# dylkot/cNMF

Measured on AMD Instinct MI355X. Metric: NMF restarts/sec (50000x2000xK5..13), higher is better.
Workload: dtype f32 (exact integer f16 plane x 2 f16 planes with per-row exponent, f32 accumulate)

## Files before the change

cnmf_amd/csrc/kernels_gemm2h.hip.h:

```cpp
#pragma once
#include <hip/hip_runtime.h>
#include "kernels_gemm3.hip.h"
#include "kernels_planes.hip.h"

namespace cnmf {

typedef _Float16 f16x8 __attribute__((ext_vector_type(8)));
typedef float f32x4_g __attribute__((ext_vector_type(4)));
typedef _Float16 f16x2_g __attribute__((ext_vector_type(2)));

#ifndef G2_U8_SKIP
#define G2_U8_SKIP 0
#endif

constexpr int G2_ROWB = 64;
constexpr int G2_A = G3_MW * G2_ROWB;
constexpr int G2_B = G3C_JW * 32;

template <int NSUB, bool HI, bool U8 = false>
struct G2Geom {
    static_assert(NSUB == 1 || (NSUB == 2 && !HI), "two blocks per step: one count plane only");
    static_assert(!U8 || NSUB == 2, "the byte plane is read by the 16x16x32 body only");
    static constexpr int IMGS = NSUB == 1 ? 4 : 3;
    static constexpr int IMG = U8 ? NSUB * G2_A + G2_B : NSUB * (G2_A + (HI ? 2 : 1) * G2_B);
    static constexpr int OFF_B = NSUB * G2_A, OFF_H = OFF_B + NSUB * G2_B;
    static constexpr int NA = NSUB * 2, NB = U8 ? 1 : NSUB;
    static constexpr int AHEAD = IMGS - 1;
    static constexpr int LDS_BYTES = IMGS * IMG;
};

template <int NSUB, bool U8 = false> struct G2Sub {};

#define G2_DMA_PIECE(NSUB_, HI_, NTB_, s_, i_)                                                     \
    {                                                                                              \
        using GEO_ = G2Geom<NSUB_, HI_>;                                                           \
        unsigned char* d_ = smem + ((s_) % GEO_::IMGS) * GEO_::IMG + wave * 1024;                  \
        if ((i_) < GEO_::NA)                                                                       \
            __builtin_amdgcn_global_load_lds(G3_AS1(abase + (size_t)(s_) * ((NSUB_) * G2_A) + (i_) * 8192), \
                                             G3_AS3(d_ + (i_) * 8192), 16, 0, 0);                  \
        else if ((i_) < GEO_::NA + GEO_::NB)    \
            __builtin_amdgcn_global_load_lds(G3_AS1(bbase + (size_t)(s_) * ((NSUB_) * G2_B) + ((i_) - GEO_::NA) * 8192), \
                                             G3_AS3(d_ + GEO_::OFF_B + ((i_) - GEO_::NA) * 8192), 16, 0, (NTB_) ? 2 : 0); \
        else if constexpr (HI_)                                                                    \
            __builtin_amdgcn_global_load_lds(G3_AS1(hbase + (size_t)(s_) * ((NSUB_) * G2_B) + ((i_) - GEO_::NA - GEO_::NB) * 8192), \
                                             G3_AS3(d_ + GEO_::OFF_H + ((i_) - GEO_::NA - GEO_::NB) * 8192), 16, 0, (NTB_) ? 2 : 0); \
    }

template <bool PART>
__device__ __forceinline__ unsigned g2_wave_live(unsigned live, int grp)
{
    return PART ? (unsigned)__builtin_amdgcn_readfirstlane((int)((live >> (grp * 4)) & 0xfu)) : 0xfu;
}


template <int VAR, bool NTB, bool PART, bool U8 = false>
__device__ __forceinline__ void gemm2h_segment_mf16(const unsigned char* __restrict__ A2, const unsigned char* __restrict__ B1,
                                                    const float* __restrict__ rscale, int Kb, float* __restrict__ C,
                                                    int ldc, int m0, int j0, int kb0, int nkb, unsigned char* smem,
                                                    unsigned live)
{
    static_assert(VAR == 0 || VAR == 2 || VAR == 3 || VAR == 4 || VAR == 6 || VAR == 7, "instruction streams 1 and 5 were retired");
    static_assert(!U8 || VAR == 0 || VAR == 4, "the byte plane has the burst and the spread stream only");
    using GEO = G2Geom<2, false, U8>;
    constexpr int NSUB = 2, IMGS = GEO::IMGS, IMG = GEO::IMG, OFF_B = GEO::OFF_B, NA = GEO::NA, NB = GEO::NB, AHEAD = GEO::AHEAD;
    constexpr bool BURST = VAR == 0, NOMFMA = VAR == 2, NODMA = VAR == 3 || VAR == 6 || VAR == 7;
    constexpr bool NOREAD = VAR == 6 || VAR == 7, NOBAR = VAR == 7;
    static_assert(IMGS == 3 && NA + NB == (U8 ? 5 : 6), "three images, six pieces per step (bytes: five)");
    const int tid = threadIdx.x;
    const int lane = tid & 63, wave = tid >> 6;
    const int grp = wave >> 2, wn = wave & 3;
    const int r = lane & 15, g = lane >> 4;
    const int ub = g >> 1, hf = g & 1;
    const int nst = nkb / NSUB;
    const unsigned lv = g2_wave_live<PART>(live, grp);
#define G2_LIVE(mt_) (!PART || ((lv >> ((mt_) >> 1)) & 1u))

    const unsigned char* abase = A2 + ((size_t)(m0 / G3_MW) * Kb + kb0) * G2_A + tid * 16;
    const unsigned char* bbase = U8 ? B1 + ((size_t)(j0 / G3C_JW) * (Kb / NSUB) + kb0 / NSUB) * G2_B + tid * 16
                                    : B1 + ((size_t)(j0 / G3C_JW) * Kb + kb0) * G2_B + tid * 16;
    constexpr const unsigned char* hbase = nullptr;

    f32x4_g acc[8][4];
#pragma unroll
    for (int mt = 0; mt < 8; ++mt)
#pragma unroll
        for (int nt = 0; nt < 4; ++nt)
#pragma unroll
            for (int i = 0; i < 4; ++i) acc[mt][nt][i] = 0.f;

    const int a_row = ub * G2_A + (grp * 128 + r) * G2_ROWB;
    const int a_s0 = ((0 + hf) ^ ((r >> 2) & 3)) * 16, a_s1 = ((2 + hf) ^ ((r >> 2) & 3)) * 16;
    const int b_off = U8 ? OFF_B + wn * 2048 + lane * 16 : OFF_B + ub * G2_B + (wn * 64 + r) * 32 + (hf ^ ((r >> 3) & 1)) * 16;

#define G2_DMA_PIECE_U8(s_, i_)                                                                    \
    {                                                                                              \
        unsigned char* d_ = smem + ((s_) % IMGS) * IMG + wave * 1024;                              \
        if ((i_) < NA)                                                                             \
            __builtin_amdgcn_global_load_lds(G3_AS1(abase + (size_t)(s_) * (NSUB * G2_A) + (i_) * 8192), \
                                             G3_AS3(d_ + (i_) * 8192), 16, 0, 0);                  \
        else                                                                                       \
            __builtin_amdgcn_global_load_lds(G3_AS1(bbase + (size_t)(s_) * G2_B), G3_AS3(d_ + OFF_B), 16, 0, NTB ? 2 : 0); \
    }
#define G2_PIECE(s_, i_) { if constexpr (U8) G2_DMA_PIECE_U8(s_, i_) else G2_DMA_PIECE(2, false, NTB, s_, i_) __builtin_amdgcn_sched_barrier(0); }
#define G2_SPOT(MORE_, p_)                                                                         \
    if (!BURST && MORE_) {                                                                         \
        if constexpr (!U8) G2_PIECE(s + AHEAD, p_)                                                 \
        else if constexpr ((p_) != G2_U8_SKIP) G2_PIECE(s + AHEAD, (p_) < G2_U8_SKIP ? (p_) : (p_) - 1) \
    }
#define G2_CVT2(w_, sel_) __builtin_bit_cast(unsigned, __builtin_bit_cast(f16x2_g, __builtin_amdgcn_perm(0x64646464u, (w_), (sel_))) - f16x2_g{(_Float16)1024.0f, (_Float16)1024.0f})
#define G2_SEL_LO 0x04010400u
#define G2_SEL_HI 0x04030402u
#define G2_CVT(nt_)                                                                                \
    {                                                                                              \
        const unsigned w0_ = braw[(nt_) >> 1][2 * ((nt_) & 1)], w1_ = braw[(nt_) >> 1][2 * ((nt_) & 1) + 1]; \
        u32x4 c_;                                                                                  \
        c_.x = G2_CVT2(w0_, G2_SEL_LO); c_.y = G2_CVT2(w0_, G2_SEL_HI);                            \
        c_.z = G2_CVT2(w1_, G2_SEL_LO); c_.w = G2_CVT2(w1_, G2_SEL_HI);                            \
        bq[nt_] = __builtin_bit_cast(f16x8, c_);                                                   \
    }
#define G2_ISSUE(s_) { _Pragma("unroll") for (int i = 0; i < NA + NB; ++i) G2_PIECE(s_, i) }
#define G2_FRAG(ptr_) __builtin_bit_cast(f16x8, *reinterpret_cast<const u32x4*>(ptr_))
#define G2_AFRAG(bb_, mt_, q_) G2_FRAG((bb_) + a_row + (mt_) * 16 * G2_ROWB + ((q_) ? a_s1 : a_s0))
#define G2_READ_A(s_)                                                                              \
    {                                                                                              \
        const unsigned char* bb = smem + ((s_) % IMGS) * IMG;                                      \
        if constexpr (U8) { _Pragma("unroll") for (int p = 0; p < 2; ++p) braw[p] = *reinterpret_cast<const u32x4*>(bb + b_off + p * 1024); } \
        else { _Pragma("unroll") for (int nt = 0; nt < 4; ++nt) bq[nt] = G2_FRAG(bb + b_off + nt * 16 * 32); } \
        _Pragma("unroll") for (int mp = 0; mp < 4; mp += 2) {                                      \
            aq[mp][1] = G2_AFRAG(bb, mp, 1); aq[mp + 1][1] = G2_AFRAG(bb, mp + 1, 1);              \
            aq[mp][0] = G2_AFRAG(bb, mp, 0); aq[mp + 1][0] = G2_AFRAG(bb, mp + 1, 0);              \
        }                                                                                          \
        __builtin_amdgcn_sched_barrier(0);                                                         \
         \
        if constexpr (U8) { _Pragma("unroll") for (int nt = 0; nt < 4; ++nt) G2_CVT(nt) }          \
    }
#define G2_READ_B(s_)                                                                              \
    {                                                                                              \
        const unsigned char* bb = smem + ((s_) % IMGS) * IMG;                                      \
        _Pragma("unroll") for (int mp = 4; mp < 8; mp += 2) {                                      \
            aq[mp][1] = G2_AFRAG(bb, mp, 1); aq[mp + 1][1] = G2_AFRAG(bb, mp + 1, 1);              \
            aq[mp][0] = G2_AFRAG(bb, mp, 0); aq[mp + 1][0] = G2_AFRAG(bb, mp + 1, 0);              \
        }                                                                                          \
        __builtin_amdgcn_sched_barrier(0);                                                         \
    }
#define G2_MF(mt_, q_)                                                                             \
    if constexpr (NOMFMA) { asm volatile("" :: "v"(aq[mt_][q_]), "v"(bq[0]), "v"(bq[1]), "v"(bq[2]), "v"(bq[3])); } \
    else if (G2_LIVE(mt_)) {                                                                       \
        _Pragma("unroll") for (int nt = 0; nt < 4; ++nt)                                           \
            acc[mt_][nt] = __builtin_amdgcn_mfma_f32_16x16x32_f16(aq[mt_][q_], bq[nt], acc[mt_][nt], 0, 0, 0); \
    }
#define G2_MF8(ma_, mb_, q_) G2_MF(ma_, q_) G2_MF(mb_, q_)
#define G2_STEP(MORE_)                                                                             \
    {                                                                                              \
        if constexpr (!NOBAR) G3_RAW_BARRIER()                   \
        if (BURST && MORE_) G2_ISSUE(s + AHEAD)                                                    \
        if constexpr (NOREAD) { if (s == 0) { G2_READ_A(s) G2_READ_B(s) } } else { G2_READ_A(s) }  \
        G2_MF8(0, 1, 1)                                                                            \
        G2_SPOT(MORE_, 0)                                                                          \
        G2_MF8(0, 1, 0)                                                                            \
        if constexpr (!NOREAD) { G2_READ_B(s) }                                                    \
        G2_SPOT(MORE_, 1)                                                                          \
        G2_MF8(2, 3, 1)                                                                            \
        G2_SPOT(MORE_, 2)                                                                          \
        G2_MF8(2, 3, 0)                                                                            \
        asm volatile("s_waitcnt lgkmcnt(0)" ::: "memory");       \
                                          \
        if (s + 1 < nst) {                                                                         \
            if (MORE_) {                                                                           \
                if constexpr (U8) { if constexpr (BURST) G3_WAIT_VM(5); else if constexpr (G2_U8_SKIP < 3) G3_WAIT_VM(2); else G3_WAIT_VM(3); } \
                else { if constexpr (BURST) G3_WAIT_VM(6); else G3_WAIT_VM(3); }                   \
            } else G3_WAIT_VM(0);                                                                  \
        }                                                                                          \
        if constexpr (!NOBAR) G3_RAW_BARRIER()                                            \
        G2_MF8(4, 5, 1)                                                                            \
        G2_SPOT(MORE_, 3)                                                                          \
        G2_MF8(4, 5, 0)                                                                            \
        G2_SPOT(MORE_, 4)                                                                          \
        G2_MF8(6, 7, 1)                                                                            \
        G2_SPOT(MORE_, 5)                                                                          \
        G2_MF8(6, 7, 0)                                                                            \
    }

    f16x8 bq[4], aq[8][2];
    u32x4 braw[2];
    G3_WAIT_VM(0);
    G2_ISSUE(0)
    if (nst > 1) G2_ISSUE(1)
    if (nst > 1) { if constexpr (U8) G3_WAIT_VM(5); else G3_WAIT_VM(6); } else G3_WAIT_VM(0);
    if (grp == 1) G3_RAW_BARRIER()
    {
        int s = 0;
        const int n_main = NODMA ? 0 : nst - AHEAD;
        for (; s < n_main; ++s) G2_STEP(true)
        for (; s < nst; ++s) G2_STEP(false)
    }
    if (grp == 0) G3_RAW_BARRIER()
#undef G2_STEP
#undef G2_MF8
#undef G2_MF
#undef G2_READ_B
#undef G2_READ_A
#undef G2_AFRAG
#undef G2_FRAG
#undef G2_ISSUE
#undef G2_CVT
#undef G2_SEL_HI
#undef G2_SEL_LO
#undef G2_CVT2
#undef G2_SPOT
#undef G2_PIECE
#undef G2_DMA_PIECE_U8

    if (C == nullptr) return;
#pragma unroll
    for (int mt = 0; mt < 8; ++mt) {
        if (!G2_LIVE(mt)) continue;
        const int row0 = m0 + grp * 128 + mt * 16 + 4 * g;
#pragma unroll
        for (int i = 0; i < 4; ++i) {
            const float rs = rscale[row0 + i];
#pragma unroll
            for (int nt = 0; nt < 4; ++nt)
                C[(size_t)(row0 + i) * ldc + j0 + wn * 64 + nt * 16 + r] = acc[mt][nt][i] * rs;
        }
    }
#undef G2_LIVE
}

template <bool HI, int VAR, bool NTB, bool PART, bool GEN>
__device__ __forceinline__ void gemm2h_segment(G2Sub<1>, const unsigned char* __restrict__ A2, const unsigned char* __restrict__ B1,
                                                   const unsigned char* __restrict__ Bhi,
                                                   const unsigned int* __restrict__ hiflag,
                                                   const float* __restrict__ rscale,
                                                   int Kb, float* __restrict__ C, int ldc, int m0, int j0, int kb0,
                                                   int nkb, unsigned char* smem, const float* __restrict__ cscale,
                                                   unsigned live)
{
    static_assert(VAR == 0 || VAR == 4, "the 32x32x16 body has the burst and the spread stream only");
    using GEO = G2Geom<1, HI>;
    constexpr int IMGS = GEO::IMGS, IMG = GEO::IMG, OFF_B = GEO::OFF_B, AHEAD = GEO::AHEAD;
    static_assert(IMGS == 4 && GEO::NA == 2 && GEO::NB == 1, "four images, pieces A0 A1 B (Bhi)");
    const int tid = threadIdx.x;
    const int lane = tid & 63, wave = tid >> 6;
    const int grp = wave >> 2, wn = wave & 3;
    const int li = lane & 31, h = lane >> 5;
    const int nst = nkb;
    const unsigned lv = g2_wave_live<PART>(live, grp);
#define G2_LIVE(m_) (!PART || ((lv >> (m_)) & 1u))

    const size_t jblk = ((size_t)(j0 / G3C_JW) * Kb + kb0);
    const unsigned char* abase = A2 + ((size_t)(m0 / G3_MW) * Kb + kb0) * G2_A + tid * 16;
    const unsigned char* bbase = B1 + jblk * G2_B + tid * 16;
    const unsigned char* hbase = HI ? Bhi + jblk * G2_B + tid * 16 : nullptr;
    unsigned int fw[5] = {0u, 0u, 0u, 0u, 0u};
    if (HI) {
        const int KW = (Kb + 31) >> 5, w0 = kb0 >> 5;
        const unsigned int* fr = hiflag + (size_t)(j0 / G3C_JW) * KW;
#pragma unroll
        for (int w = 0; w < 5; ++w)
            fw[w] = (nkb > 129) ? 0xFFFFFFFFu : ((w0 + w < KW) ? __builtin_amdgcn_readfirstlane(fr[w0 + w]) : 0u);
    }
    const int fbit0 = kb0 & 31;

    f32x16_3 acc[4][2];
#pragma unroll
    for (int m = 0; m < 4; ++m)
#pragma unroll
        for (int n = 0; n < 2; ++n)
#pragma unroll
            for (int r = 0; r < 16; ++r) acc[m][n][r] = 0.f;

    const int a_row = (grp * 128 + li) * G2_ROWB;
    const int a_s0 = ((0 + h) ^ ((li >> 2) & 3)) * 16, a_s1 = ((2 + h) ^ ((li >> 2) & 3)) * 16;
    const int b_off = OFF_B + (wn * 64 + li) * 32 + (h ^ ((li >> 3) & 1)) * 16;

#define G2_BLKFLAG(b_) (HI && ((fw[(fbit0 + (b_)) >> 5 > 4 ? 4 : (fbit0 + (b_)) >> 5] >> ((fbit0 + (b_)) & 31)) & 1u))
#define G2_ISSUE(s_)                                                                               \
    {                                                                                              \
        unsigned char* d_ = smem + ((s_) % IMGS) * IMG + wave * 1024;                              \
        const unsigned char* a_ = abase + (size_t)(s_) * G2_A;                                     \
        _Pragma("unroll") for (int i = 0; i < 2; ++i)                                              \
            __builtin_amdgcn_global_load_lds(G3_AS1(a_ + i * 8192), G3_AS3(d_ + i * 8192), 16, 0, 0); \
        __builtin_amdgcn_global_load_lds(G3_AS1(bbase + (size_t)(s_) * G2_B), G3_AS3(d_ + OFF_B), 16, 0, NTB ? 2 : 0); \
        if (HI) {                                                                                  \
            if (G2_BLKFLAG(s_))                                                                    \
                __builtin_amdgcn_global_load_lds(G3_AS1(hbase + (size_t)(s_) * G2_B), G3_AS3(d_ + GEO::OFF_H), 16, 0, NTB ? 2 : 0); \
        }                                                                                          \
    }
#define G2_PIECE(s_, i_) { G2_DMA_PIECE(1, HI, NTB, s_, i_) __builtin_amdgcn_sched_barrier(0); }
#define G2_FRAG(ptr_) __builtin_bit_cast(f16x8, *reinterpret_cast<const u32x4*>(ptr_))
#define G2_MFMA(b_, m_, q_)                                                                        \
    if (G2_LIVE(m_)) {                                                                             \
    acc[m_][0] = __builtin_amdgcn_mfma_f32_32x32x16_f16(aq[m_][q_], b_[0], acc[m_][0], 0, 0, 0);   \
    acc[m_][1] = __builtin_amdgcn_mfma_f32_32x32x16_f16(aq[m_][q_], b_[1], acc[m_][1], 0, 0, 0); }
#define G2_WAIT_AHEAD(cnt_)                                                                        \
    {                                                                                              \
        if constexpr ((cnt_) == 1) G3_WAIT_VM(3);                                                  \
        else if constexpr ((cnt_) == 2) G3_WAIT_VM(6);                                             \
        else G3_WAIT_VM(0);                                                                        \
    }

    f16x8 bq[2], bh[2], aq[4][2];
    constexpr bool SPREAD = VAR == 4 && (!HI || GEN);
    G3_WAIT_VM(0);
    G2_ISSUE(0)
    if (nst > 1) G2_ISSUE(1)
    if (nst > 2) G2_ISSUE(2)
    if (nst > 2) G2_WAIT_AHEAD(2) else if (nst > 1) G2_WAIT_AHEAD(1) else G2_WAIT_AHEAD(0)
    if (grp == 1) G3_RAW_BARRIER()
    if constexpr (SPREAD) {
#define G2_READ_A(s_)                                                                              \
        {                                                                                          \
            const unsigned char* bb = smem + ((s_) % IMGS) * IMG;                                  \
            _Pragma("unroll") for (int n = 0; n < 2; ++n) bq[n] = G2_FRAG(bb + b_off + n * 32 * 32); \
            _Pragma("unroll") for (int m = 0; m < 2; ++m) {                                        \
                aq[m][1] = G2_FRAG(bb + a_row + m * 32 * G2_ROWB + a_s1);                          \
                aq[m][0] = G2_FRAG(bb + a_row + m * 32 * G2_ROWB + a_s0);                          \
            }                                                                                      \
            if constexpr (HI) { _Pragma("unroll") for (int n = 0; n < 2; ++n) bh[n] = G2_FRAG(bb + b_off + G2_B + n * 32 * 32); } \
            __builtin_amdgcn_sched_barrier(0);                                                     \
        }
#define G2_READ_B(s_)                                                                              \
        {                                                                                          \
            const unsigned char* bb = smem + ((s_) % IMGS) * IMG;                                  \
            _Pragma("unroll") for (int m = 2; m < 4; ++m) {                                        \
                aq[m][1] = G2_FRAG(bb + a_row + m * 32 * G2_ROWB + a_s1);                          \
                aq[m][0] = G2_FRAG(bb + a_row + m * 32 * G2_ROWB + a_s0);                          \
            }                                                                                      \
            __builtin_amdgcn_sched_barrier(0);                                                     \
        }
#define G2_STEP(MORE_)                                                                             \
        {                                                                                          \
            G3_RAW_BARRIER()                                         \
            G2_READ_A(s)                                                                           \
            G2_MFMA(bq, 0, 1) G2_MFMA(bq, 1, 1)                                                    \
            if (MORE_) G2_PIECE(s + AHEAD, 0)                                                      \
            G2_MFMA(bq, 0, 0) G2_MFMA(bq, 1, 0)                                                    \
            G2_READ_B(s)                                                                           \
            if (MORE_) G2_PIECE(s + AHEAD, 1)                                                      \
            if constexpr (HI) { G2_MFMA(bh, 0, 0) G2_MFMA(bh, 1, 0) }                              \
            asm volatile("s_waitcnt lgkmcnt(0)" ::: "memory");                                     \
             \
            if (s + 1 < nst) { if (MORE_) { if constexpr (HI) G3_WAIT_VM(6); else G3_WAIT_VM(5); } else G3_WAIT_VM(0); } \
            G3_RAW_BARRIER()                                                              \
            G2_MFMA(bq, 2, 1) G2_MFMA(bq, 3, 1)                                                    \
            if (MORE_) G2_PIECE(s + AHEAD, 2)                                                      \
            G2_MFMA(bq, 2, 0) G2_MFMA(bq, 3, 0)                                                    \
            if constexpr (HI) { if (MORE_) G2_PIECE(s + AHEAD, 3)                                  \
                                G2_MFMA(bh, 2, 0) G2_MFMA(bh, 3, 0) }                              \
        }
        {
            int s = 0;
            const int n_main = nst - AHEAD;
            for (; s < n_main; ++s) G2_STEP(true)
            for (; s < nst; ++s) G2_STEP(false)
        }
#undef G2_STEP
#undef G2_READ_B
#undef G2_READ_A
    } else {
#define G2_READ(s_)                                                                                \
        {                                                                                          \
            const unsigned char* bb = smem + ((s_) % IMGS) * IMG;                                  \
            _Pragma("unroll") for (int n = 0; n < 2; ++n) bq[n] = G2_FRAG(bb + b_off + n * 32 * 32); \
            if (HI) { _Pragma("unroll") for (int n = 0; n < 2; ++n) bh[n] = G2_FRAG(bb + b_off + G2_B + n * 32 * 32); } \
            _Pragma("unroll") for (int m = 0; m < 4; ++m) {                                        \
                aq[m][0] = G2_FRAG(bb + a_row + m * 32 * G2_ROWB + a_s0);                          \
                aq[m][1] = G2_FRAG(bb + a_row + m * 32 * G2_ROWB + a_s1);                          \
            }                                                                                      \
            __builtin_amdgcn_sched_barrier(0);                                                     \
        }
#define G2_MFMA4(b_, ma_, mb_) G2_MFMA(b_, ma_, 1) G2_MFMA(b_, mb_, 1) G2_MFMA(b_, ma_, 0) G2_MFMA(b_, mb_, 0)
#define G2_MFMA2H(b_, ma_, mb_) G2_MFMA(b_, ma_, 0) G2_MFMA(b_, mb_, 0)
#define G2_HALF(ma_, mb_)                                                                          \
        {                                                                                          \
            G2_MFMA4(bq, ma_, mb_)                                                                 \
            if (HI) { if (hi_blk) { if constexpr (GEN) { G2_MFMA2H(bh, ma_, mb_) } else { G2_MFMA4(bh, ma_, mb_) } } } \
        }
        for (int s = 0; s < nst; ++s) {
            const bool hi_blk = G2_BLKFLAG(s);
            G3_RAW_BARRIER()
            if (s + AHEAD < nst) G2_ISSUE(s + AHEAD)
            G2_READ(s)
            G2_HALF(0, 1)
            asm volatile("s_waitcnt lgkmcnt(0)" ::: "memory");
            if (s + 1 < nst) {
                if (s + 3 < nst) G2_WAIT_AHEAD(2) else if (s + 2 < nst) G2_WAIT_AHEAD(1) else G2_WAIT_AHEAD(0)
            }
            G3_RAW_BARRIER()
            G2_HALF(2, 3)
        }
#undef G2_HALF
#undef G2_MFMA2H
#undef G2_MFMA4
#undef G2_READ
    }
    if (grp == 0) G3_RAW_BARRIER()
#undef G2_WAIT_AHEAD
#undef G2_MFMA
#undef G2_FRAG
#undef G2_PIECE
#undef G2_ISSUE
#undef G2_BLKFLAG

    if (C == nullptr) return;
    const int j = j0 + wn * 64 + li;
    const float cs[2] = {(HI && cscale) ? cscale[j] : 1.0f, (HI && cscale) ? cscale[j + 32] : 1.0f};
#pragma unroll
    for (int m = 0; m < 4; ++m) {
        if (!G2_LIVE(m)) continue;
        const int cbase = m0 + grp * 128 + m * 32 + 4 * h;
#pragma unroll
        for (int n = 0; n < 2; ++n)
#pragma unroll
            for (int r = 0; r < 16; ++r) {
                const int row = cbase + (r & 3) + 8 * (r >> 2);
                C[(size_t)row * ldc + j + n * 32] = (acc[m][n][r] * rscale[row]) * cs[n];
            }
    }
#undef G2_LIVE
}

template <bool HI, int VAR, bool NTB, bool PART, bool GEN, bool U8>
__device__ __forceinline__ void gemm2h_segment(G2Sub<2, U8>, const unsigned char* __restrict__ A2, const unsigned char* __restrict__ B1,
                                               const unsigned char* __restrict__, const unsigned int* __restrict__,
                                               const float* __restrict__ rscale, int Kb, float* __restrict__ C, int ldc,
                                               int m0, int j0, int kb0, int nkb, unsigned char* smem, const float* __restrict__,
                                               unsigned live)
{
    static_assert(!HI && !GEN, "two blocks per step: one count plane only");
    gemm2h_segment_mf16<VAR, NTB, PART, U8>(A2, B1, rscale, Kb, C, ldc, m0, j0, kb0, nkb, smem, live);
}

template <int NSUB, bool HI, int VAR = 0, bool PART = false, bool GEN = false, bool U8 = false>
__global__ __launch_bounds__(512) void gemm2h_kernel(const unsigned char* __restrict__ A2,
                                                     const unsigned char* __restrict__ B1,
                                                     const unsigned char* __restrict__ Bhi,
                                                     const unsigned int* __restrict__ hiflag,
                                                     const float* __restrict__ rscale, int Kb,
                                                     float* __restrict__ C, int ldc, long long c_split_stride,
                                                     int kb_per, const float* __restrict__ cscale = nullptr,
                                                     unsigned long long livemask = ~0ull)
{
    extern __shared__ __attribute__((aligned(16))) unsigned char smem3[];
    int jt = blockIdx.x, mg = blockIdx.y, z = blockIdx.z;
    if ((gridDim.z & 7) == 0) {
        const int L = blockIdx.x + (int)gridDim.x * (blockIdx.y + (int)gridDim.y * blockIdx.z);
        const int xcd = L & 7, idx = L >> 3;
        jt = idx % (int)gridDim.x;
        mg = (idx / (int)gridDim.x) % (int)gridDim.y;
        z = xcd + 8 * (idx / (int)(gridDim.x * gridDim.y));
    }
    const int kb0 = z * kb_per;
    const int nkb = min(kb_per, Kb - kb0);
    gemm2h_segment<HI, VAR, true, PART, GEN>(G2Sub<NSUB, U8>{}, A2, B1, Bhi, hiflag, rscale, Kb, C ? C + (size_t)z * c_split_stride : nullptr, ldc, mg * G3_MW,
                                                   jt * G3C_JW, kb0, nkb, smem3, cscale, (unsigned)((livemask >> (8 * mg)) & 0xffu));
}

template <int NSUB, bool HI, int VAR = 0, bool NTB = true, bool PART = false, bool GEN = false, bool U8 = false>
__global__ __launch_bounds__(512) void gemm2h_streamk_kernel(const unsigned char* __restrict__ A2,
                                                             const unsigned char* __restrict__ B1,
                                                             const unsigned char* __restrict__ Bhi,
                                                             const unsigned int* __restrict__ hiflag,
                                                             const float* __restrict__ rscale, int Kb,
                                                             float* __restrict__ C0, float* __restrict__ C1,
                                                             float* __restrict__ C2, int ldc, int MG, int T, int xmap,
                                                             const float* __restrict__ cscale = nullptr,
                                                             unsigned long long livemask = ~0ull)
{
    extern __shared__ __attribute__((aligned(16))) unsigned char smem3[];
    const int Ks = Kb / NSUB;
    const long long U = (long long)T * Ks;
    const int P = (int)gridDim.x;
    const int q = (xmap && MG > 1 && P % MG == 0) ? ((int)blockIdx.x % MG) * (P / MG) + (int)blockIdx.x / MG : (int)blockIdx.x;
    long long u = U * q / P;
    const long long u1 = U * (q + 1) / P;
    const int NJ = T / MG;
    while (u < u1) {
        const int tile = (int)(u / Ks), ks = (int)(u % Ks);
        const int ke = (int)min((long long)Ks, ks + (u1 - u));
        const int mg = tile / NJ, jt = tile % NJ;
        gemm2h_segment<HI, VAR, NTB, PART, GEN>(G2Sub<NSUB, U8>{}, A2, B1, Bhi, hiflag, rscale, Kb, (ks == 0) ? C0 : (ke == Ks ? C1 : C2), ldc, mg * G3_MW,
                                                      jt * G3C_JW, ks * NSUB, (ke - ks) * NSUB, smem3, cscale,
                                                      (unsigned)((livemask >> (8 * mg)) & 0xffu));
        u += ke - ks;
        G3_WAIT_VM(0);
        __syncthreads();
    }
}

}
```

Before: 236.5.

## Permute MFMA fragment rows to remove LDS bank conflicts in the 16x16 gemm body

Adds a constexpr helper header that models ds_read_b128 bank conflicts and defines permuted row mappings for the factor and count fragments. The 16x16x32 body now reads LDS rows through these permutations, and the epilogue remaps output rows and columns to match. The default U8 skip piece also changes from 0 to 2. The aim is fewer LDS bank conflicts on fragment reads. The cost is extra index arithmetic and a scattered output store pattern, and correctness depends on the permutation being consistent between reads and writes.

New measurement: 238.8 (median of 6 runs). Within noise of the previous version (+1.0%).

```diff
diff --git a/cnmf_amd/csrc/g2_frag.h b/cnmf_amd/csrc/g2_frag.h
--- /dev/null
+++ b/cnmf_amd/csrc/g2_frag.h
@@ -0,0 +1,76 @@
+#pragma once
+
+#include <cstdint>
+
+namespace g2frag {
+
+constexpr int ROWB = 64, A_BYTES = 256 * ROWB, B_BYTES = 256 * 32;
+constexpr int MF16_OFF_B = 2 * A_BYTES;
+constexpr int M32_OFF_B = A_BYTES;
+
+constexpr int b128_lane_group(int lane)
+{
+    const int l = lane & 31;
+    const bool first = l < 4 || (l >= 12 && l < 16) || (l >= 20 && l < 28);
+    return (lane >> 5) * 2 + (first ? 0 : 1);
+}
+
+template <class Off>
+constexpr int b128_extra_cycles(Off off)
+{
+    int extra = 0;
+    for (int grp = 0; grp < 4; ++grp) {
+        int worst = 0;
+        for (int bank = 0; bank < 16; ++bank) {
+            int addr[16] = {}, n = 0;
+            for (int lane = 0; lane < 64; ++lane) {
+                if (b128_lane_group(lane) != grp) continue;
+                const int a = off(lane);
+                if (((a >> 4) & 15) != bank) continue;
+                bool seen = false;
+                for (int i = 0; i < n; ++i) seen = seen || addr[i] == a;
+                if (!seen) addr[n++] = a;
+            }
+            worst = n > worst ? n : worst;
+        }
+        extra += worst - 1;
+    }
+    return extra;
+}
+
+constexpr int mf16_sigma(int t) { return (0x1320 >> (4 * t)) & 3; }
+constexpr int mf16_factor_row(int r) { return 4 * mf16_sigma(r >> 2) + (r & 3); }
+constexpr int mf16_count_row(int r) { return r ^ ((r & 8) >> 1); }
+
+constexpr int mf16_factor_off(int lane, int grp, int mt, int q, bool permuted = true)
+{
+    const int r = lane & 15, g = lane >> 4, ub = g >> 1, hf = g & 1;
+    const int row = permuted ? mf16_factor_row(r) : r;
+    return ub * A_BYTES + (grp * 128 + mt * 16 + row) * ROWB + (((2 * q + hf) ^ ((row >> 2) & 3)) * 16);
+}
+
+constexpr int mf16_count_off(int lane, int wn, int nt, bool permuted = true)
+{
+    const int r = lane & 15, g = lane >> 4, ub = g >> 1, hf = g & 1;
+    const int row = permuted ? mf16_count_row(r) : r;
+    return MF16_OFF_B + ub * B_BYTES + (wn * 64 + nt * 16 + row) * 32 + ((hf ^ ((row >> 3) & 1)) * 16);
+}
+
+constexpr int mf16_count_u8_off(int lane, int wn, int p) { return MF16_OFF_B + wn * 2048 + p * 1024 + lane * 16; }
+
+constexpr int mf16_out_row(int g, int mt, int i) { return mt * 16 + 4 * mf16_sigma(g) + i; }
+constexpr int mf16_out_col(int r, int nt, bool u8) { return nt * 16 + (u8 ? r : mf16_count_row(r)); }
+
+constexpr int m32_factor_off(int lane, int grp, int m, int q)
+{
+    const int li = lane & 31, h = lane >> 5;
+    return (grp * 128 + m * 32 + li) * ROWB + (((2 * q + h) ^ ((li >> 2) & 3)) * 16);
+}
+
+constexpr int m32_count_off(int lane, int wn, int n, int plane)
+{
+    const int li = lane & 31, h = lane >> 5;
+    return M32_OFF_B + plane * B_BYTES + (wn * 64 + n * 32 + li) * 32 + ((h ^ ((li >> 3) & 1)) * 16);
+}
+
+}
diff --git a/cnmf_amd/csrc/kernels_gemm2h.hip.h b/cnmf_amd/csrc/kernels_gemm2h.hip.h
--- a/cnmf_amd/csrc/kernels_gemm2h.hip.h
+++ b/cnmf_amd/csrc/kernels_gemm2h.hip.h
@@ -2,6 +2,7 @@
 #include <hip/hip_runtime.h>
 #include "kernels_gemm3.hip.h"
 #include "kernels_planes.hip.h"
+#include "g2_frag.h"
 
 namespace cnmf {
 
@@ -10,12 +11,17 @@
 typedef _Float16 f16x2_g __attribute__((ext_vector_type(2)));
 
 #ifndef G2_U8_SKIP
-#define G2_U8_SKIP 0
+#define G2_U8_SKIP 2
+#endif
+
+#ifndef G2_U8_PERMUTE
+#define G2_U8_PERMUTE 1
 #endif
 
 constexpr int G2_ROWB = 64;
 constexpr int G2_A = G3_MW * G2_ROWB;
 constexpr int G2_B = G3C_JW * 32;
+static_assert(g2frag::ROWB == G2_ROWB && g2frag::A_BYTES == G2_A && g2frag::B_BYTES == G2_B, "g2_frag.h restates this geometry");
 
 template <int NSUB, bool HI, bool U8 = false>
 struct G2Geom {
@@ -88,9 +94,12 @@
 #pragma unroll
             for (int i = 0; i < 4; ++i) acc[mt][nt][i] = 0.f;
 
-    const int a_row = ub * G2_A + (grp * 128 + r) * G2_ROWB;
-    const int a_s0 = ((0 + hf) ^ ((r >> 2) & 3)) * 16, a_s1 = ((2 + hf) ^ ((r >> 2) & 3)) * 16;
-    const int b_off = U8 ? OFF_B + wn * 2048 + lane * 16 : OFF_B + ub * G2_B + (wn * 64 + r) * 32 + (hf ^ ((r >> 3) & 1)) * 16;
+    constexpr bool PERM = !U8 || G2_U8_PERMUTE;
+    const int pr = PERM ? g2frag::mf16_factor_row(r) : r;
+    const int pc = U8 ? r : g2frag::mf16_count_row(r);
+    const int a_row = ub * G2_A + (grp * 128 + pr) * G2_ROWB;
+    const int a_s0 = ((0 + hf) ^ ((pr >> 2) & 3)) * 16, a_s1 = ((2 + hf) ^ ((pr >> 2) & 3)) * 16;
+    const int b_off = U8 ? OFF_B + wn * 2048 + lane * 16 : OFF_B + ub * G2_B + (wn * 64 + pc) * 32 + (hf ^ ((pc >> 3) & 1)) * 16;
 
 #define G2_DMA_PIECE_U8(s_, i_)                                                                    \
     {                                                                                              \
@@ -215,13 +224,13 @@
 #pragma unroll
     for (int mt = 0; mt < 8; ++mt) {
         if (!G2_LIVE(mt)) continue;
-        const int row0 = m0 + grp * 128 + mt * 16 + 4 * g;
+        const int row0 = m0 + grp * 128 + mt * 16 + 4 * (PERM ? g2frag::mf16_sigma(g) : g);
 #pragma unroll
         for (int i = 0; i < 4; ++i) {
             const float rs = rscale[row0 + i];
 #pragma unroll
             for (int nt = 0; nt < 4; ++nt)
-                C[(size_t)(row0 + i) * ldc + j0 + wn * 64 + nt * 16 + r] = acc[mt][nt][i] * rs;
+                C[(size_t)(row0 + i) * ldc + j0 + wn * 64 + nt * 16 + pc] = acc[mt][nt][i] * rs;
         }
     }
 #undef G2_LIVE
```
